# huangjh-pub/di-fusion

Measured on AMD Instinct MI355X. Metric: frames/s integrate+decode+mesh, 640x480 synthetic stream, higher is better.
Workload: dtype f32

## Files before the change

### di_fusion_amd/csrc/kernels_extract.hip.h

```cpp
#pragma once

__device__ __forceinline__ void mark_confident_nbhd(const Geo& g, int lin, float ignore_th, const int64_t* __restrict__ indexer,
                                                    const float* __restrict__ obs, const GridMarks& marks) {
    const uint32_t* bits = marks.bits;
    int ix, iy, iz;
    unlinearize(g, lin, ix, iy, iz);
    int cand[7];
    cand[0] = lin;
    cand[1] = linearize(g, clampi(ix - 1, 0, g.nx - 1), iy, iz);
    cand[2] = linearize(g, clampi(ix + 1, 0, g.nx - 1), iy, iz);
    cand[3] = linearize(g, ix, clampi(iy - 1, 0, g.ny - 1), iz);
    cand[4] = linearize(g, ix, clampi(iy + 1, 0, g.ny - 1), iz);
    cand[5] = linearize(g, ix, iy, clampi(iz - 1, 0, g.nz - 1));
    cand[6] = linearize(g, ix, iy, clampi(iz + 1, 0, g.nz - 1));
    int64_t slot[7];
#pragma unroll
    for (int c = 0; c < 7; ++c) slot[c] = indexer[cand[c]];
    float w[7];
#pragma unroll
    for (int c = 0; c < 7; ++c) w[c] = slot[c] >= 0 ? obs[slot[c]] : ignore_th;
    uint32_t word[7];
#pragma unroll
    for (int c = 0; c < 7; ++c) word[c] = (w[c] > ignore_th) ? bits[cand[c] >> 5] : 0xFFFFFFFFu;
    uint32_t prev[7];
// ... 248 lines not shown
            float xn, yn, zn; int ix, iy, iz;
            bool ok = voxel_of(A.geo, pose_row(A.pose, 0, x, y, z), pose_row(A.pose, 1, x, y, z), pose_row(A.pose, 2, x, y, z), xn, yn, zn, ix, iy, iz);
            int64_t slot = -1;
            if (ok) {
                slot = A.indexer[linearize(A.geo, ix, iy, iz)];
                ok = slot >= 0 && A.obs[slot] > A.ignore_th;
            }
            R.live = ok;
            R.out_idx = row;
            if (ok) {
                R.px = (xn - (float)ix) - 0.5f; R.py = (yn - (float)iy) - 0.5f; R.pz = (zn - (float)iz) - 0.5f;
                lat_row = A.latent + slot * L;
            } else if (half == 1) A.out_std[row] = 0.0f;
        }
    } else {
        const int64_t row = tile * 32 + col;
        R.live = row < n_rows;
        if (R.live) {
            const int64_t p = A.list[row];
            float xn, yn, zn; int ix, iy, iz;
            voxel_of(A.geo, A.xyz[p * 3 + 0], A.xyz[p * 3 + 1], A.xyz[p * 3 + 2], xn, yn, zn, ix, iy, iz);
            R.px = (xn - (float)ix) - 0.5f; R.py = (yn - (float)iy) - 0.5f; R.pz = (zn - (float)iz) - 0.5f;
            lat_row = A.latent + A.indexer[linearize(A.geo, ix, iy, iz)] * L;
            R.out_idx = row;
        }
    }
#pragma unroll
    for (int t = 0; t < 16; ++t) {
        const int k = 2 * t + half;
        float v = 0.0f;
        if (R.live) {
            if (row32) v = row32[k];
            else if (k < L) v = lat_row[k];
            else v = (k == L) ? R.px : ((k == L + 1) ? R.py : R.pz);
        }
        xin[t] = v;
    }
    if constexpr (!DENSE) {
        if (A.mode == 2) {
            unsigned nf = 0;
#pragma unroll
            for (int t = 0; t < 16; ++t) nf |= ((__float_as_uint(xin[t]) & 0x7f800000u) == 0x7f800000u) ? 1u : 0u;
            nf |= (unsigned)__shfl_xor((int)nf, 32);
            R.bad = nf != 0;
        }
    }
    return R;
}

template <bool GRAD, bool DENSE = false>
__global__ void __launch_bounds__(GRAD ? 256 : 512, GRAD ? 1 : 2) k_decode(DecodeArgs A, const float* __restrict__ wblob) {
    extern __shared__ __attribute__((aligned(16))) float lds[];
    if (DENSE && A.zero_word && blockIdx.x == 0 && threadIdx.x == 0) *A.zero_word = 0;
    stage_weights(lds, wblob, DEC_LDS_FLOATS);
    const __amdgpu_buffer_rsrc_t wfwd = make_rsrc(wblob, DEC_FLOATS);
    const __amdgpu_buffer_rsrc_t wbwd = make_rsrc(GRAD ? A.wbwd : wblob, GRAD ? DECB_FLOATS : DEC_FLOATS);
    const int lane = lane_id(), half = lane >> 5, col = lane & 31;
    const int wave = (int)((threadIdx.x >> 6) * gridDim.x + blockIdx.x);
    const int nwaves = (int)(gridDim.x * (blockDim.x >> 6));
    const int res3 = A.lat.res * A.lat.res * A.lat.res;
    const int tiles_per_voxel = (res3 + 31) / 32;
    int64_t n_rows, n_tiles;
    if (A.mode == 0) {
        n_rows = (int64_t)(*A.n_ptr) * res3;
        n_tiles = (int64_t)(*A.n_ptr) * tiles_per_voxel;
    } else {
        n_rows = A.n_ptr ? (int64_t)(*A.n_ptr) : A.n_static;
        n_tiles = (n_rows + 31) / 32;
    }
    for (int64_t tile = wave; tile < n_tiles; tile += nwaves) {
        f16v xin;
        const DecodeRow R = decode_row_input<DENSE>(A, tile, col, half, res3, tiles_per_voxel, n_rows, xin);
        const bool live = R.live;
        const int64_t out_idx = R.out_idx;
        const float px = R.px, py = R.py, pz = R.pz;
        float sdf, sd;
        if (!GRAD && A.mode == 1 && A.fold_table) {
            const int b = live ? A.list[tile * 32 + col] / res3 : 0;
            decoder_tile_folded(lds, wfwd, FoldInitGlobal{A.fold_table + (int64_t)b * 256}, px, py, pz, lane, sdf, sd);
        } else if (GRAD) {
            float gx, gy, gz;
            decoder_tile_grad(lds, wfwd, wbwd, xin, lane, sdf, sd, gx, gy, gz);
            if (live && half == 1) {
                const float gs = R.bad ? __builtin_nanf("") : A.grad_scale;
                A.out_grad[out_idx * 3 + 0] = gx * gs;
                A.out_grad[out_idx * 3 + 1] = gy * gs;
                A.out_grad[out_idx * 3 + 2] = gz * gs;
            }
        } else {
            decoder_tile(lds, wfwd, xin, lane, sdf, sd);
        }
        if (live) {
            if (half == 0) A.out_sdf[out_idx] = R.bad ? __builtin_nanf("") : A.sign * sdf;
            else A.out_std[out_idx] = R.bad ? __builtin_nanf("") : sd;
        }
    }
}

template <bool DENSE = false>
__global__ void __launch_bounds__(512, 1) k_decode_x6(DecodeArgs A, const float* __restrict__ wblob, const float* __restrict__ wu) {
    extern __shared__ __attribute__((aligned(16))) float lds[];
    if (DENSE && A.zero_word && blockIdx.x == 0 && threadIdx.x == 0) *A.zero_word = 0;
    stage_weights(lds, wblob, X6_LDS_BYTES / 4);
    const __amdgpu_buffer_rsrc_t wfwd = make_rsrc(wblob, X6_BYTES / 4);
    const __amdgpu_buffer_rsrc_t wun = make_rsrc(wu, X6U_BYTES / 4);
    const int lane = lane_id(), half = lane >> 5, col = lane & 31;
    const int wave = (int)((threadIdx.x >> 6) * gridDim.x + blockIdx.x);
    const int nwaves = (int)(gridDim.x * (blockDim.x >> 6));
    const int res3 = A.lat.res * A.lat.res * A.lat.res;
    const int tiles_per_voxel = (res3 + 31) / 32;
    int64_t n_rows, n_tiles;
    if (A.mode == 0) {
        n_rows = (int64_t)(*A.n_ptr) * res3;
        n_tiles = (int64_t)(*A.n_ptr) * tiles_per_voxel;
    } else {
        n_rows = A.n_ptr ? (int64_t)(*A.n_ptr) : A.n_static;
        n_tiles = (n_rows + 31) / 32;
    }
    for (int64_t tile = wave; tile < n_tiles; tile += nwaves) {
        f16v xin;
        const DecodeRow R = decode_row_input<DENSE>(A, tile, col, half, res3, tiles_per_voxel, n_rows, xin);
        const bool live = R.live;
        const int64_t out_idx = R.out_idx;
        float sdf, sd;
        decoder_tile_x6(lds, wfwd, wun, xin, lane, sdf, sd);
        if (live) {
            if (half == 0) A.out_sdf[out_idx] = R.bad ? __builtin_nanf("") : A.sign * sdf;
            else A.out_std[out_idx] = R.bad ? __builtin_nanf("") : sd;
        }
    }
}

#ifndef GRAD_X6_THREADS
#define GRAD_X6_THREADS 256
#endif
template <int PF, bool DENSE = false>
__global__ void __launch_bounds__(GRAD_X6_THREADS, 1) k_decode_grad_x6(DecodeArgs A, const float* __restrict__ wblob, const float* __restrict__ wu,
                                                          const float* __restrict__ wb) {
    extern __shared__ __attribute__((aligned(16))) float lds[];
    if (DENSE && A.zero_word && blockIdx.x == 0 && threadIdx.x == 0) *A.zero_word = 0;
    stage_weights(lds, wblob, X6_LDS_BYTES / 4);
    const __amdgpu_buffer_rsrc_t wfwd = make_rsrc(wblob, X6_BYTES / 4);
    const __amdgpu_buffer_rsrc_t wun = make_rsrc(wu, X6U_BYTES / 4);
    const __amdgpu_buffer_rsrc_t wbw = make_rsrc(wb, X6B_BYTES / 4);
    const int lane = lane_id(), half = lane >> 5, col = lane & 31;
    const int wave = (int)((threadIdx.x >> 6) * gridDim.x + blockIdx.x);
    const int nwaves = (int)(gridDim.x * (blockDim.x >> 6));
    const int res3 = A.lat.res * A.lat.res * A.lat.res;
    const int64_t n_rows = A.n_ptr ? (int64_t)(*A.n_ptr) : A.n_static;
    const int64_t n_tiles = (n_rows + 31) / 32;
    for (int64_t tile = wave; tile < n_tiles; tile += nwaves) {
        f16v xin;
        const DecodeRow R = decode_row_input<DENSE>(A, tile, col, half, res3, 1, n_rows, xin);
        float sdf, sd, gx, gy, gz;
        decoder_tile_grad_x6<PF>(lds, wfwd, wun, wbw, xin, lane, sdf, sd, gx, gy, gz);
        if (R.live) {
            if (half == 0) A.out_sdf[R.out_idx] = R.bad ? __builtin_nanf("") : A.sign * sdf;
            else {
                const float gs = R.bad ? __builtin_nanf("") : A.grad_scale;
                A.out_std[R.out_idx] = R.bad ? __builtin_nanf("") : sd;
                A.out_grad[R.out_idx * 3 + 0] = gx * gs;
                A.out_grad[R.out_idx * 3 + 1] = gy * gs;
                A.out_grad[R.out_idx * 3 + 2] = gz * gs;
            }
        }
    }
}

template <int NS>
__device__ __forceinline__ void decode_refine_x6_body(const BatchN<DecodeArgs, NS>& B, int S, const float* __restrict__ wblob) {
    extern __shared__ __attribute__((aligned(16))) float lds[];
    const int lane = lane_id(), half = lane >> 5, col = lane & 31;
    const int wave = __builtin_amdgcn_readfirstlane((int)((threadIdx.x >> 6) * gridDim.x + blockIdx.x));
    const int nwaves = (int)(gridDim.x * (blockDim.x >> 6));
    const Lattice lat = B.s[0].lat;
    const float sign = B.s[0].sign;
    const int res3 = lat.res * lat.res * lat.res, r = lat.res;
    Ranges<NS, int64_t> rg;
    rg.pre[0] = 0;
#pragma unroll
    for (int j = 0; j < NS; ++j) {
        rg.cnt[j] = (j < S) ? (B.s[j].n_ptr ? (int64_t)(*B.s[j].n_ptr) : B.s[j].n_static) : 0;
        rg.pre[j + 1] = rg.pre[j] + (rg.cnt[j] + 31) / 32;
    }
    const int64_t n_tiles = rg.total();
    int sm_n; int64_t lt_n, rows_n;
    rg.locate(wave, sm_n, lt_n, rows_n);
    int e_next = (wave < n_tiles && lt_n * 32 + col < rows_n) ? B.s[sm_n].list[lt_n * 32 + col] : 0;
    __builtin_amdgcn_sched_barrier(0);
    stage_weights(lds, wblob, X6_LDS_BYTES / 4);
    const __amdgpu_buffer_rsrc_t wfwd = make_rsrc(wblob, X6_BYTES / 4);
    for (int64_t T = wave; T < n_tiles; T += nwaves) {
        const int sm = sm_n;
        const int64_t tile = lt_n, n_rows = rows_n;
        const DecodeArgs& A = B.s[sm];
        const int64_t row = tile * 32 + col;
        const bool live = row < n_rows;
        const int e = e_next;
        rg.locate(T + nwaves, sm_n, lt_n, rows_n);
        e_next = (T + nwaves < n_tiles && lt_n * 32 + col < rows_n) ? B.s[sm_n].list[lt_n * 32 + col] : 0;
        const int b = e / res3, sb = e - b * res3;
        const float px = lat.coord(sb / (r * r)), py = lat.coord((sb / r) % r), pz = lat.coord(sb % r);
        float sdf, sd;
// ... 64 lines not shown
                cube_sdf[e0 + jz] = -sv;
                cube_std[e0 + jz] = dv;
                if (fabsf(sv) < 0.05f) sel |= 1u << jz;
            }
        }
        int total;
        int ex = block_excl_scan(__popc(sel), smem, total);
        if (total > 0) {
            if (threadIdx.x == 0) s_base = atomicAdd(counters + DIF_C_VH, total);
            __syncthreads();
            int o = s_base + ex;
            while (sel) {
                int jz = __ffs((int)sel) - 1;
                sel &= sel - 1;
                refine_list[o++] = (int32_t)(e0 + jz);
            }
        }
        __syncthreads();
    }
}

struct VoxelDecodeArgs {
    const int32_t* occ_slot;
    const float* latent;
    Lattice low;
    int R;
    float* cube_sdf;
    float* cube_std;
    int32_t* refine_list;
    int* counters;
    const float* fold_w;
    float* fold_table;
};

#define VD_MAX_L3 64
#define VD_MAX_R2 64
#define VD_WAVE_LDS_FLOATS (2 * VD_MAX_L3 + 2 * 256)

#ifdef DIF_TRACE
__device__ unsigned long long g_vd_trace[2048 * 8];
#define VD_STAMP(slot) do { if (lane_id() == 0) g_vd_trace[((threadIdx.x >> 6) * gridDim.x + blockIdx.x) * 8 + (slot)] = wall_clock64(); } while (0)
#else
#define VD_STAMP(slot) do { } while (0)
#endif

template <bool X6, int NS>
__device__ __forceinline__ void decode_voxels_body(const BatchN<VoxelDecodeArgs, NS>& AB, int S, const float* __restrict__ wblob) {
    extern __shared__ __attribute__((aligned(16))) float lds[];
    VD_STAMP(0);
    constexpr int LDS_W = X6 ? X6_LDS_BYTES / 4 : ((DEC_LDS_FLOATS + 3) & ~3);
#if defined(DIF_VD_CUT) && DIF_VD_CUT == 0
    return;
#endif
    stage_weights(lds, wblob, X6 ? X6_LDS_BYTES / 4 : DEC_LDS_FLOATS);
    VD_STAMP(1);
#if defined(DIF_VD_CUT) && DIF_VD_CUT == 1
    return;
#endif
    const __amdgpu_buffer_rsrc_t wfwd = make_rsrc(wblob, X6 ? X6_BYTES / 4 : DEC_FLOATS);
    const int lane = lane_id(), half = lane >> 5, col = lane & 31, wid = threadIdx.x >> 6;
    const int pair = wid >> 1, tsel = wid & 1;
    float* w_low_sdf = lds + LDS_W + pair * VD_WAVE_LDS_FLOATS;
    float* w_low_std = w_low_sdf + VD_MAX_L3;
    float* w_fold = w_low_std + VD_MAX_L3 + tsel * 256;
    const Lattice low = AB.s[0].low;
    const float* const fold_w = AB.s[0].fold_w;
    const int l = low.res, R = AB.s[0].R, l3 = l * l * l, R2 = R * R, R3 = R2 * R;
    const float scale = (float)(l - 1) / (float)(R - 1);
    int pre[NS + 1];
    pre[0] = 0;
#pragma unroll
    for (int j = 0; j < NS; ++j) pre[j + 1] = pre[j] + ((j < S) ? AB.s[j].counters[DIF_C_B] : 0);
    const int B = pre[NS];
    const int pairs_per_block = (int)(blockDim.x >> 7), n_pairs = (int)gridDim.x * pairs_per_block;
    const int first = __builtin_amdgcn_readfirstlane(pair * (int)gridDim.x + (int)blockIdx.x);
    __shared__ int s_tot[8], s_map[8], s_base[NS];
    const int rounds = (B + n_pairs - 1) / n_pairs;
    for (int round = 0; round < rounds; ++round) {
        const int bg = first + round * n_pairs;
        int sm = 0, b = bg;
#pragma unroll
        for (int j = 1; j < NS; ++j)
            if (bg >= pre[j]) { sm = j; b = bg - pre[j]; }
        const VoxelDecodeArgs& A = AB.s[sm];
        unsigned sel = 0;
        const int jz0 = tsel * (R >> 1), jz1 = jz0 + (R >> 1);
        const int64_t e0 = (int64_t)b * R3 + (int64_t)lane * R;
        if (bg < B && tsel * 32 < l3) {
            const float* lat_row = A.latent + (int64_t)A.occ_slot[b] * L;
            const int s = tsel * 32 + col;
            const float px = low.coord(s / (l * l)), py = low.coord((s / l) % l), pz = low.coord(s % l);
            float sdf = 0.0f, sd = 0.0f;
            if (X6 || fold_w) {
                if constexpr (X6) decoder_fold_consts_x6(lds, fold_w, lat_row, w_fold, lane);
                else decoder_fold_consts(lds, fold_w, lat_row, w_fold, lane);
                __builtin_amdgcn_wave_barrier();
                __builtin_amdgcn_s_waitcnt(0xc07f);
                if (tsel == 0) {
                    float* rec = A.fold_table + (int64_t)b * 256;
                    for (int p = lane; p < 256; p += 64) rec[p] = w_fold[p];
                }
                VD_STAMP(6);
#if defined(DIF_VD_CUT) && DIF_VD_CUT == 2
                sdf = w_fold[lane]; sd = w_fold[lane + 64];
#else
                if constexpr (X6) decoder_tile_folded_x6(lds, wfwd, FoldInitLds{w_fold}, px, py, pz, lane, sdf, sd);
                else decoder_tile_folded(lds, wfwd, FoldInitLds{w_fold}, px, py, pz, lane, sdf, sd);
#endif
            } else if constexpr (!X6) {
                f16v xin;
#pragma unroll
                for (int t = 0; t < 16; ++t) {
                    const int k = 2 * t + half;
                    xin[t] = (k < L) ? lat_row[k] : 0.0f;
                }
                if (half) { xin[14] = px; xin[15] = pz; } else { xin[15] = py; }
                decoder_tile(lds, wfwd, xin, lane, sdf, sd);
            }
            if (s < l3) {
                if (half == 0) w_low_sdf[s] = sdf;
                else w_low_std[s] = sd;
            }
        }
        __syncthreads();
        VD_STAMP(2);
        if (bg < B && lane < R2) {
            const int jx = lane / R, jy = lane % R;
            int x0, x1, y0, y1; float wx0, wx1, wy0, wy1;
            tri_axis(jx, l, scale, x0, x1, wx0, wx1);
            tri_axis(jy, l, scale, y0, y1, wy0, wy1);
            float* const cube_sdf = A.cube_sdf;
            float* const cube_std = A.cube_std;
            for (int jz = jz0; jz < jz1; ++jz) {
                int z0, z1; float wz0, wz1;
                tri_axis(jz, l, scale, z0, z1, wz0, wz1);
                float sv = tri_sample(w_low_sdf, l, x0, x1, y0, y1, z0, z1, wx0, wx1, wy0, wy1, wz0, wz1);
                float dv = tri_sample(w_low_std, l, x0, x1, y0, y1, z0, z1, wx0, wx1, wy0, wy1, wz0, wz1);
                cube_sdf[e0 + jz] = -sv;
                cube_std[e0 + jz] = dv;
                if (fabsf(sv) < 0.05f) sel |= 1u << jz;
            }
        }
        VD_STAMP(3);
        const int c = __popc(sel);
        const int incl = wave_incl_scan(c);
        const int total = __shfl(incl, 63);
        if (lane == 0) { s_tot[wid] = total; if (NS > 1) s_map[wid] = sm; }
        __syncthreads();
        if (NS == 1) {
            if (threadIdx.x == 0) {
                int sum = 0;
                for (int w = 0; w < (int)(blockDim.x >> 6); ++w) sum += s_tot[w];
                s_base[0] = sum ? atomicAdd(A.counters + DIF_C_VH, sum) : 0;
            }
        } else if ((int)threadIdx.x < S) {
            const int j = (int)threadIdx.x;
            int sum = 0;
            for (int w = 0; w < (int)(blockDim.x >> 6); ++w) sum += (s_map[w] == j) ? s_tot[w] : 0;
            s_base[j] = sum ? atomicAdd(AB.s[j].counters + DIF_C_VH, sum) : 0;
        }
        __syncthreads();
        if (total > 0) {
// ... 25 lines not shown
```

### di_fusion_amd/csrc/kernels_optimize.hip.h

```cpp
#pragma once

struct OptimSet {
    const float* obs; const uint8_t* optimized; const int64_t* pos; float enc_th;
    __device__ __forceinline__ bool has(int64_t slot) const { return slot >= 0 && obs[slot] >= enc_th && !optimized[slot] && pos[slot] > 0; }
};

__global__ void __launch_bounds__(DIF_BLOCK) k_optim_focus(Geo g, OptimSet S, const float* __restrict__ xyz, const uint8_t* __restrict__ unq_mask, int64_t N,
                                                         const int64_t* __restrict__ indexer, uint8_t* __restrict__ focus, int* __restrict__ counters) {
    const int64_t i = (int64_t)blockIdx.x * blockDim.x + threadIdx.x;
    if (i == 0) { counters[DIF_C_OPT_ROWS] = 0; counters[DIF_C_OPT_VOXELS] = 0; }
    if (i >= N) return;
    float xn, yn, zn; int ix, iy, iz;
    bool f = false;
    if (unq_mask[i] && voxel_of(g, xyz[i * 3 + 0], xyz[i * 3 + 1], xyz[i * 3 + 2], xn, yn, zn, ix, iy, iz)) {
        const int lin = linearize(g, ix, iy, iz), plane = g.ny * g.nz;
        const int nl[7] = {lin, lin - plane, lin + plane, lin - g.nz, lin + g.nz, lin - 1, lin + 1};
        const bool in_grid[7] = {true, ix > 0, ix < g.nx - 1, iy > 0, iy < g.ny - 1, iz > 0, iz < g.nz - 1};
#pragma unroll
        for (int q = 0; q < 7; ++q) f |= in_grid[q] && S.has(indexer[nl[q]]);
    }
    focus[i] = f ? 1 : 0;
}

struct OptimGatherFunctor {
// ... 6 lines not shown
        i = j - (int64_t)o * N;
        if (!focus[i]) return -1;
        float xn, yn, zn; int ix, iy, iz;
        voxel_of(g, xyz[i * 3 + 0], xyz[i * 3 + 1], xyz[i * 3 + 2], xn, yn, zn, ix, iy, iz);
        const float ox = (o & 4) ? 0.5f : -0.5f, oy = (o & 2) ? 0.5f : -0.5f, oz = (o & 1) ? 0.5f : -0.5f;
        const float gx = fminf(fmaxf(ceilf(xn + ox) - 1.0f, 0.0f), (float)(g.nx - 1));
        const float gy = fminf(fmaxf(ceilf(yn + oy) - 1.0f, 0.0f), (float)(g.ny - 1));
        const float gz = fminf(fmaxf(ceilf(zn + oz) - 1.0f, 0.0f), (float)(g.nz - 1));
        rx = (xn - gx) - 0.5f; ry = (yn - gy) - 0.5f; rz = (zn - gz) - 0.5f;
        const int64_t slot = indexer[linearize(g, (int)gx, (int)gy, (int)gz)];
        return S.has(slot) ? slot : -1;
    }
    __device__ int count(int j) const { float a, b, c; int64_t i; return neighbour(j, a, b, c, i) >= 0 ? 1 : 0; }
    __device__ void emit(int j, int k) const {
        float rx, ry, rz; int64_t i;
        const int64_t slot = neighbour(j, rx, ry, rz, i);
        const float sdf = noise[k] * 0.05f;
        row_slot[k] = (int)slot;
        row_xyz[(int64_t)k * 3 + 0] = rx + sdf * normal[i * 3 + 0];
        row_xyz[(int64_t)k * 3 + 1] = ry + sdf * normal[i * 3 + 1];
        row_xyz[(int64_t)k * 3 + 2] = rz + sdf * normal[i * 3 + 2];
        row_sdf[k] = sdf;
        slot_flag[slot] = 1;
    }
    __device__ void finish(int total) const { counters[DIF_C_OPT_ROWS] = total; }
};

struct OptimUniqueFunctor {
    const int* slot_flag; int* slot_u; int* uniq_slot; int* counters;
    __device__ int count(int s) const { return slot_flag[s] ? 1 : 0; }
    __device__ void emit(int s, int u) const { uniq_slot[u] = s; slot_u[s] = u; }
    __device__ void finish(int total) const { counters[DIF_C_OPT_VOXELS] = total; }
};

#define DIF_OPT_FIX_SCALE 1099511627776.0f

__global__ void __launch_bounds__(DIF_BLOCK) k_optim_init(const int* __restrict__ uniq_slot, const float* __restrict__ latent, float* __restrict__ z,
                                                        float* __restrict__ m, float* __restrict__ v, long long* __restrict__ grad,
                                                        const int* __restrict__ counters) {
    const int n = counters[DIF_C_OPT_VOXELS] * 32;
    for (int e = blockIdx.x * blockDim.x + threadIdx.x; e < n; e += gridDim.x * blockDim.x) {
        const int u = e >> 5, f = e & 31;
        z[e] = f < L ? latent[(int64_t)uniq_slot[u] * L + f] : 0.0f;
        m[e] = 0.0f; v[e] = 0.0f; grad[e] = 0;
    }
}

template <bool X6>
__global__ void __launch_bounds__(256, 1) k_optim_grad(const float* __restrict__ wblob, const float* __restrict__ wbwd_blob, const float* __restrict__ wu_blob, const int* __restrict__ row_slot,
                                                     const float* __restrict__ row_xyz, const float* __restrict__ row_sdf, const int* __restrict__ slot_u,
                                                     const float* __restrict__ z, unsigned long long* __restrict__ grad, float* __restrict__ loss_sum,
                                                     const int* __restrict__ counters) {
    extern __shared__ __attribute__((aligned(16))) float lds[];
    stage_weights(lds, wblob, X6 ? X6_LDS_BYTES / 4 : DEC_LDS_FLOATS);
    const __amdgpu_buffer_rsrc_t wfwd = make_rsrc(wblob, X6 ? X6_BYTES / 4 : DEC_FLOATS), wbwd = make_rsrc(wbwd_blob, X6 ? X6B_BYTES / 4 : DECB_FLOATS);
    const __amdgpu_buffer_rsrc_t wun = make_rsrc(X6 ? wu_blob : wblob, X6 ? X6U_BYTES / 4 : 4);
    const int lane = lane_id(), half = lane >> 5, col = lane & 31;
    const int wave = (int)((threadIdx.x >> 6) * gridDim.x + blockIdx.x), nwaves = (int)(gridDim.x * (blockDim.x >> 6));
    const int n_rows = counters[DIF_C_OPT_ROWS];
    const float inv_n = 1.0f / (float)n_rows;
    const int n_tiles = (n_rows + 31) >> 5;
    for (int tile = wave; tile < n_tiles; tile += nwaves) {
        const int row = tile * 32 + col;
        const bool live = row < n_rows;
        const int u = live ? slot_u[row_slot[row]] : -1;
        const float* zr = z + (int64_t)(live ? u : 0) * 32;
        f16v xin;
#pragma unroll
        for (int t = 0; t < 16; ++t) {
            const int k = 2 * t + half;
            float val = 0.0f;
            if (live) val = k < L ? zr[k] : row_xyz[(int64_t)row * 3 + (k - L)];
            xin[t] = val;
        }
        float sdf, sd, loss;
        f16v gx;
        if constexpr (X6) decoder_tile_nll_grad_x6<GRAD_X6_PF>(lds, wfwd, wun, wbwd, xin, lane, live ? row_sdf[row] : 0.0f, inv_n, sdf, sd, loss, gx);
        else decoder_tile_nll_grad(lds, wfwd, wbwd, xin, lane, live ? row_sdf[row] : 0.0f, inv_n, sdf, sd, loss, gx);
        const int u_prev = __shfl_up(u, 1), u_next = __shfl_down(u, 1);
        const bool run_head = (col == 0) || (u_prev != u), run_tail = (col == 31) || (u_next != u);
        const uint32_t heads32 = (uint32_t)(__ballot(run_head) >> (half * 32));
        const int my_head = 31 - __clz((int)(heads32 & ((2u << col) - 1u)));
#pragma unroll
        for (int r = 0; r < 16; ++r) {
            long long q = live ? __float2ll_rn(gx[r] * DIF_OPT_FIX_SCALE) : 0ll;
            q = seg_incl_scan32(q, col, my_head);
            const int f = (r & 3) + 8 * (r >> 2) + 4 * half;
            if (live && run_tail && f < L) (void)__hip_atomic_fetch_add(grad + (int64_t)u * 32 + f, (unsigned long long)q, __ATOMIC_RELAXED, __HIP_MEMORY_SCOPE_AGENT);
        }
        if (loss_sum) {
            float ls = (live && half == 0) ? loss : 0.0f;
#pragma unroll
            for (int d = 32; d >= 1; d >>= 1) ls += __shfl_xor(ls, d);
            if (lane == 0) atomicAdd(loss_sum, ls);
        }
    }
}

__global__ void __launch_bounds__(DIF_BLOCK) k_optim_adam(float* __restrict__ z, float* __restrict__ m, float* __restrict__ v, long long* __restrict__ grad,
                                                        const int* __restrict__ counters, int iter, float lr, float reg_lambda) {
    const int n_vox = counters[DIF_C_OPT_VOXELS];
    const float inv_n = 1.0f / (float)counters[DIF_C_OPT_ROWS];
    const int grp = (int)((blockIdx.x * blockDim.x + threadIdx.x) >> 5), ngrp = (int)((gridDim.x * blockDim.x) >> 5), f = threadIdx.x & 31;
    const float b1 = 0.9f, b2 = 0.999f, eps = 1e-8f;
    const float step = lr / (1.0f - powf(b1, (float)iter)), bc2 = sqrtf(1.0f - powf(b2, (float)iter));
    for (int u = grp; u < n_vox; u += ngrp) {
        const int e = u * 32 + f;
        const float zf = z[e];
        float g = (float)grad[e] * (1.0f / DIF_OPT_FIX_SCALE);
        grad[e] = 0;
        if (reg_lambda > 0.0f) {
            float nn = f < L ? zf * zf : 0.0f;
// ... 24 lines not shown
```

### di_fusion_amd/csrc/mlp.hip.h

```cpp
#pragma once
#include "common.hip.h"

namespace dif {

typedef float f16v __attribute__((ext_vector_type(16)));
typedef float f4v __attribute__((ext_vector_type(4)));

__device__ __forceinline__ f16v mfma32(float a, float b, f16v c) { return __builtin_amdgcn_mfma_f32_32x32x2f32(a, b, c, 0, 0, 0); }

__device__ __forceinline__ f16v load_bias16(const float* b, int half) {
    const f4v* p = reinterpret_cast<const f4v*>(b + half * 16);
    f4v b0 = p[0], b1 = p[1], b2 = p[2], b3 = p[3];
    f16v r;
    r[0] = b0.x; r[1] = b0.y; r[2] = b0.z; r[3] = b0.w;
    r[4] = b1.x; r[5] = b1.y; r[6] = b1.z; r[7] = b1.w;
    r[8] = b2.x; r[9] = b2.y; r[10] = b2.z; r[11] = b2.w;
    r[12] = b3.x; r[13] = b3.y; r[14] = b3.z; r[15] = b3.w;
    return r;
}

__device__ __forceinline__ float relu1(float x) { return __int_as_float(max(__float_as_int(x), 0)); }
__device__ __forceinline__ f16v relu16(f16v v) {
#pragma unroll
    for (int i = 0; i < 16; ++i) v[i] = relu1(v[i]);
// ... 130 lines not shown
                                             const f16v& xin, int lane, float& sdf, float& stdv) {
    const int half = lane >> 5;
    f16v hx[1];
    hx[0] = xin;
    f16v h0[4];
#pragma unroll
    for (int mb = 0; mb < 4; ++mb) {
        f16v acc = load_bias16(W + DEC_B0 + mb * 32, half);
        acc = block_mm<1>(reinterpret_cast<const f4v*>(W + DEC_A0) + (mb * 4) * 64, hx, acc, lane);
        h0[mb] = relu16(acc);
    }
    f16v h1[4];
#pragma unroll
    for (int mb = 0; mb < 4; ++mb) {
        f16v acc = load_bias16(W + DEC_B1 + mb * 32, half);
        acc = block_mm<4>(reinterpret_cast<const f4v*>(W + DEC_A1) + (mb * 16) * 64, h0, acc, lane);
        h1[mb] = relu16(acc);
    }
    f16v h2x[4];
#pragma unroll
    for (int mb = 0; mb < 3; ++mb) {
        f16v acc = load_bias16(W + DEC_B2 + mb * 32, half);
        acc = block_mm<4>(reinterpret_cast<const f4v*>(W + DEC_A2) + (mb * 16) * 64, h1, acc, lane);
        h2x[mb] = relu16(acc);
    }
    h2x[3] = xin;
    int off3 = DEC_A3 * 4;
    asm volatile("" : "+s"(off3) : : "memory");
    float ps = 0.0f, pu = 0.0f;
#pragma unroll
    for (int mb = 0; mb < 4; ++mb) {
        f16v acc = load_bias16(W + DEC_B3 + mb * 32, half);
        acc = block_mm_src<4>(BufA{Wg, off3 + mb * 16 * 1024}, h2x, acc, lane);
        acc = relu16(acc);
        f16v ws = load_bias16(W + DEC_HW + mb * 32, half);
        f16v wu = load_bias16(W + DEC_HU + mb * 32, half);
#pragma unroll
        for (int r = 0; r < 16; ++r) {
            ps = fmaf(acc[r], ws[r], ps);
            pu = fmaf(acc[r], wu[r], pu);
        }
    }
    ps += __shfl_xor(ps, 32);
    pu += __shfl_xor(pu, 32);
    ps += W[DEC_HB + 0];
    pu += W[DEC_HB + 1];
    sdf = tanhf(ps);
    float sp = (pu > 20.0f) ? pu : log1pf(expf(pu));
    stdv = 0.05f + 0.5f * sp;
}

#define DECF_FLOATS (2 * 29 * 128)

template <int B0, int B3, int UNROLL>
__device__ __forceinline__ void decoder_fold_consts_at(const float* __restrict__ W , const float* __restrict__ fold ,
                                                       const float* __restrict__ lat_row, float* __restrict__ c, int lane) {
    float a0 = W[B0 + lane], a1 = W[B0 + lane + 64], a2 = W[B3 + lane], a3 = W[B3 + lane + 64];
    const f4v* wk = reinterpret_cast<const f4v*>(fold) + lane;
#pragma unroll UNROLL
    for (int k = 0; k < 29; ++k) {
        const float zk = lat_row[k];
        const f4v wv = wk[k * 64];
        a0 = fmaf(wv.x, zk, a0);
        a1 = fmaf(wv.y, zk, a1);
        a2 = fmaf(wv.z, zk, a2);
        a3 = fmaf(wv.w, zk, a3);
    }
    c[lane] = a0;
    c[lane + 64] = a1;
    c[128 + lane] = a2;
    c[128 + lane + 64] = a3;
}
__device__ __forceinline__ void decoder_fold_consts(const float* __restrict__ W, const float* __restrict__ fold, const float* __restrict__ lat_row,
                                                    float* __restrict__ c, int lane) {
    decoder_fold_consts_at<DEC_B0, DEC_B3, 8>(W, fold, lat_row, c, lane);
}

struct FoldInitLds {
    const float* c;
    __device__ __forceinline__ f16v load(int layer, int mb, int half) const { return load_bias16(c + layer * 128 + mb * 32, half); }
};
struct FoldInitGlobal {
    const float* rec;
    __device__ __forceinline__ f16v load(int layer, int mb, int half) const { return load_bias16(rec + layer * 128 + mb * 32, half); }
};

template <class INIT>
__device__ __forceinline__ void decoder_tile_folded(const float* __restrict__ W , __amdgpu_buffer_rsrc_t Wg , const INIT& init,
                                                    float px, float py, float pz, int lane, float& sdf, float& stdv) {
    const int half = lane >> 5;
    const float b14 = half ? px : 0.0f;
    const float b15 = half ? pz : py;
    f16v h0[4];
#pragma unroll
    for (int mb = 0; mb < 4; ++mb) {
        f16v acc = init.load(0, mb, half);
        const f4v a = reinterpret_cast<const f4v*>(W + DEC_A0)[(mb * 4 + 3) * 64 + lane];
        acc = mfma32(a.z, b14, acc);
        acc = mfma32(a.w, b15, acc);
        h0[mb] = relu16(acc);
        __builtin_amdgcn_sched_barrier(0);
    }
    f16v h1[4];
#pragma unroll
    for (int mb = 0; mb < 4; ++mb) {
        f16v acc = load_bias16(W + DEC_B1 + mb * 32, half);
        acc = block_mm<4>(reinterpret_cast<const f4v*>(W + DEC_A1) + (mb * 16) * 64, h0, acc, lane);
        h1[mb] = relu16(acc);
    }
    f16v h2[3];
#pragma unroll
    for (int mb = 0; mb < 3; ++mb) {
        f16v acc = load_bias16(W + DEC_B2 + mb * 32, half);
        acc = block_mm<4>(reinterpret_cast<const f4v*>(W + DEC_A2) + (mb * 16) * 64, h1, acc, lane);
        h2[mb] = relu16(acc);
    }
    int off3 = DEC_A3 * 4;
    asm volatile("" : "+s"(off3) : : "memory");
    float ps = 0.0f, pu = 0.0f;
#pragma unroll
    for (int mb = 0; mb < 4; ++mb) {
        f16v acc = init.load(1, mb, half);
        const BufA src{Wg, off3 + mb * 16 * 1024};
        const f4v ax = src.load(15, lane);
        acc = block_mm_src<3>(src, h2, acc, lane);
        acc = mfma32(ax.z, b14, acc);
        acc = mfma32(ax.w, b15, acc);
        __builtin_amdgcn_sched_barrier(0);
// ... 67 lines not shown
__device__ __forceinline__ void layer_x6(const SRC& A, const f16v* hin, f16v* acc, int lane) {
    constexpr int NS = (KB1 - KB0) * 2 * NMO;
    Tri ring[PF];
#pragma unroll
    for (int i = 0; i < PF; ++i)
        if (i < NS) ring[i] = A.load(i, lane);
    Tri x[2], xn[2];
#pragma unroll
    for (int i = 0; i < 8; ++i) split_pair_into(hin[KB0], i >> 2, i & 3, x[i >> 2]);
#pragma unroll
    for (int kb = KB0; kb < KB1; ++kb) {
#pragma unroll
        for (int s = 0; s < 2; ++s) {
#pragma unroll
            for (int mo = 0; mo < NMO; ++mo) {
                const int u = s * NMO + mo;
                const int t = (kb - KB0) * 2 * NMO + u;
                const Tri a = ring[t % PF];
                if (t + PF < NS) ring[t % PF] = A.load(t + PF, lane);
                if (kb + 1 < KB1) {
                    constexpr int per = (8 + 2 * NMO - 1) / (2 * NMO);
#pragma unroll
                    for (int i = u * per; i < (u + 1) * per && i < 8; ++i) split_pair_into(hin[kb + 1], i >> 2, i & 3, xn[i >> 2]);
                }
                acc[mo] = step_x6(a, x[s], acc[mo]);
                __builtin_amdgcn_sched_barrier(0);
            }
        }
        if (kb + 1 < KB1) { x[0] = xn[0]; x[1] = xn[1]; }
    }
}

#ifndef X6_PF_LDS
#define X6_PF_LDS 2
#endif
#define X6_A0C 0
#define X6_B0 1024
#define X6_B1 1152
#define X6_B2 1280
#define X6_B3 1376
#define X6_HW 1504
#define X6_HU 1632
#define X6_HB 1760
#define X6_A3C 1764
#define X6_AUX_FLOATS 2788
#define X6_L1 (X6_AUX_FLOATS * 4)
#define X6_L2 (X6_L1 + 98304)
#define X6_LDS_BYTES (X6_L2 + 36864)
#define X6_L3 (X6_L2 + 73728)
#define X6_BYTES (X6_L3 + 73728)

__device__ __forceinline__ void decoder_fold_consts_x6(const float* __restrict__ aux , const float* __restrict__ fold ,
                                                       const float* __restrict__ lat_row, float* __restrict__ c, int lane) {
    decoder_fold_consts_at<X6_B0, X6_B3, 15>(aux, fold, lat_row, c, lane);
}

template <class INIT>
__device__ __forceinline__ void decoder_tile_folded_x6(const float* __restrict__ W , __amdgpu_buffer_rsrc_t Wg, const INIT& init,
                                                       float px, float py, float pz, int lane, float& sdf, float& stdv) {
    const int half = lane >> 5;
    const float b14 = half ? px : 0.0f;
    const float b15 = half ? pz : py;
    const char* Wb = reinterpret_cast<const char*>(W);
    f16v h0[4];
#pragma unroll
    for (int mb = 0; mb < 4; ++mb) {
        f16v acc = init.load(0, mb, half);
        const f4v a = reinterpret_cast<const f4v*>(W + X6_A0C)[mb * 64 + lane];
        acc = mfma32(a.z, b14, acc);
        acc = mfma32(a.w, b15, acc);
        h0[mb] = relu16(acc);
    }
    f16v h1[4];
#pragma unroll
    for (int mb = 0; mb < 4; ++mb) h1[mb] = load_bias16(W + X6_B1 + mb * 32, half);
    layer_x6<0, 4, 4, X6_PF_LDS>(LdsX6{reinterpret_cast<const u4v*>(Wb + X6_L1)}, h0, h1, lane);
#pragma unroll
    for (int mb = 0; mb < 4; ++mb) h1[mb] = relu16(h1[mb]);
    f16v h2[3];
#pragma unroll
    for (int mb = 0; mb < 3; ++mb) h2[mb] = load_bias16(W + X6_B2 + mb * 32, half);
    int goff = X6_L2 + 36864;
    asm volatile("" : "+s"(goff) : : "memory");
    layer_x6<0, 2, 3, X6_PF_LDS>(LdsX6{reinterpret_cast<const u4v*>(Wb + X6_L2)}, h1, h2, lane);
    layer_x6<2, 4, 3, 3>(BufX6{Wg, goff}, h1, h2, lane);
#pragma unroll
    for (int mb = 0; mb < 3; ++mb) h2[mb] = relu16(h2[mb]);
    f16v h3[4];
#pragma unroll
    for (int mb = 0; mb < 4; ++mb) h3[mb] = init.load(1, mb, half);
    layer_x6<0, 3, 4, 3>(BufX6{Wg, goff + 36864}, h2, h3, lane);
    float ps = 0.0f, pu = 0.0f;
#pragma unroll
    for (int mb = 0; mb < 4; ++mb) {
        f16v acc = h3[mb];
        const f4v ax = reinterpret_cast<const f4v*>(W + X6_A3C)[mb * 64 + lane];
        acc = mfma32(ax.z, b14, acc);
        acc = mfma32(ax.w, b15, acc);
        acc = relu16(acc);
        f16v ws = load_bias16(W + X6_HW + mb * 32, half);
        f16v wu = load_bias16(W + X6_HU + mb * 32, half);
#pragma unroll
        for (int r = 0; r < 16; ++r) {
            ps = fmaf(acc[r], ws[r], ps);
            pu = fmaf(acc[r], wu[r], pu);
        }
    }
// ... 472 lines not shown
#pragma unroll
    for (int mb = 0; mb < 4; ++mb) {
        f16v acc = load_bias16(W + DEC_B3 + mb * 32, half);
        acc = block_mm_src<4>(BufA{Wg, off3 + mb * 16 * 1024}, h2x, acc, lane);
        acc = relu16_mask(acc, m3[mb]);
        f16v ws = load_bias16(W + DEC_HW + mb * 32, half);
        f16v wu = load_bias16(W + DEC_HU + mb * 32, half);
#pragma unroll
        for (int r = 0; r < 16; ++r) {
            ps = fmaf(acc[r], ws[r], ps);
            pu = fmaf(acc[r], wu[r], pu);
        }
    }
    ps += __shfl_xor(ps, 32);
    pu += __shfl_xor(pu, 32);
    ps += W[DEC_HB + 0];
    pu += W[DEC_HB + 1];
    sdf = tanhf(ps);
    const float sp = (pu > 20.0f) ? pu : log1pf(expf(pu));
    stdv = 0.05f + 0.5f * sp;
    const float g = fminf(fmaxf(gt, -0.2f), 0.2f), mu = fminf(fmaxf(sdf, -0.2f), 0.2f);
    const float diff = g - mu, var = stdv * stdv;
    loss = (logf(stdv) + 0.918938533204672742f + diff * diff / (2.0f * var)) * inv_n;
    const float d_mu = (sdf >= -0.2f && sdf <= 0.2f) ? -diff / var : 0.0f;
    const float d_sigma = 1.0f / stdv - diff * diff / (var * stdv);
    const float a = inv_n * d_mu * (1.0f - sdf * sdf);
    const float b = inv_n * d_sigma * 0.5f * ((pu > 20.0f) ? 1.0f : 1.0f / (1.0f + expf(-pu)));
    f16v g3[4];
#pragma unroll
    for (int mb = 0; mb < 4; ++mb) {
        f16v ws = load_bias16(W + DEC_HW + mb * 32, half);
        f16v wu = load_bias16(W + DEC_HU + mb * 32, half);
        f16v t;
#pragma unroll
        for (int r = 0; r < 16; ++r) t[r] = a * ws[r] + b * wu[r];
        g3[mb] = apply_mask16(t, m3[mb]);
    }
    f16v g2[3];
#pragma unroll
    for (int mb = 0; mb < 3; ++mb)
        g2[mb] = apply_mask16(block_mm_src<4>(BufA{Wb, offb + DECB_T3 * 4 + mb * 16 * 1024}, g3, zero16(), lane), m2[mb]);
    f16v gskip = block_mm_src<4>(BufA{Wb, offb + DECB_T3 * 4 + 3 * 16 * 1024}, g3, zero16(), lane);
    f16v g1[4];
#pragma unroll
    for (int mb = 0; mb < 4; ++mb)
        g1[mb] = apply_mask16(block_mm_src<3>(BufA{Wb, offb + DECB_T2 * 4 + mb * 12 * 1024}, g2, zero16(), lane), m1[mb]);
    f16v g0[4];
#pragma unroll
    for (int mb = 0; mb < 4; ++mb)
        g0[mb] = apply_mask16(block_mm_src<4>(BufA{Wb, offb + DECB_T1 * 4 + mb * 16 * 1024}, g1, zero16(), lane), m0[mb]);
    gx = block_mm_src<4>(BufA{Wb, offb + DECB_T0 * 4}, g0, gskip, lane);
}

__device__ __forceinline__ void stage_weights(float* lds, const float* __restrict__ g, int n_floats) {
    const f4v* __restrict__ src = reinterpret_cast<const f4v*>(g);
    f4v* dst = reinterpret_cast<f4v*>(lds);
    const int n4 = n_floats / 4, step = (int)blockDim.x;
    int i = (int)threadIdx.x;
    for (; i + 7 * step < n4; i += 8 * step) {
        f4v v[8];
#pragma unroll
        for (int k = 0; k < 8; ++k) v[k] = src[i + k * step];
#pragma unroll
        for (int k = 0; k < 8; ++k) dst[i + k * step] = v[k];
    }
    for (; i < n4; i += step) dst[i] = src[i];
    __syncthreads();
}

}
```

Before: 10030.

## Stage decoder weights via async global_load_lds and prefetch latent rows

Weight staging into LDS now uses direct global-to-LDS loads (global_load_lds) instead of round-tripping through registers, split into an issue step and a wait step. The fused decode kernel overlaps this staging with the first latent-row and occupancy-slot fetches, and then software-pipelines the next row's latent fetch across loop iterations. It reads latents via readlane from a per-lane register. Counter reads are hoisted ahead of staging in the other kernels so their latency overlaps too. This adds manual waitcnt and scheduling barriers, which carry correctness risk if the counter encoding is wrong.

```diff
diff --git a/di_fusion_amd/csrc/kernels_extract.hip.h b/di_fusion_amd/csrc/kernels_extract.hip.h
--- a/di_fusion_amd/csrc/kernels_extract.hip.h
+++ b/di_fusion_amd/csrc/kernels_extract.hip.h
@@ -324,12 +324,6 @@
 __global__ void __launch_bounds__(GRAD ? 256 : 512, GRAD ? 1 : 2) k_decode(DecodeArgs A, const float* __restrict__ wblob) {
     extern __shared__ __attribute__((aligned(16))) float lds[];
     if (DENSE && A.zero_word && blockIdx.x == 0 && threadIdx.x == 0) *A.zero_word = 0;
-    stage_weights(lds, wblob, DEC_LDS_FLOATS);
-    const __amdgpu_buffer_rsrc_t wfwd = make_rsrc(wblob, DEC_FLOATS);
-    const __amdgpu_buffer_rsrc_t wbwd = make_rsrc(GRAD ? A.wbwd : wblob, GRAD ? DECB_FLOATS : DEC_FLOATS);
-    const int lane = lane_id(), half = lane >> 5, col = lane & 31;
-    const int wave = (int)((threadIdx.x >> 6) * gridDim.x + blockIdx.x);
-    const int nwaves = (int)(gridDim.x * (blockDim.x >> 6));
     const int res3 = A.lat.res * A.lat.res * A.lat.res;
     const int tiles_per_voxel = (res3 + 31) / 32;
     int64_t n_rows, n_tiles;
@@ -340,6 +334,12 @@
         n_rows = A.n_ptr ? (int64_t)(*A.n_ptr) : A.n_static;
         n_tiles = (n_rows + 31) / 32;
     }
+    stage_weights(lds, wblob, DEC_LDS_FLOATS);
+    const __amdgpu_buffer_rsrc_t wfwd = make_rsrc(wblob, DEC_FLOATS);
+    const __amdgpu_buffer_rsrc_t wbwd = make_rsrc(GRAD ? A.wbwd : wblob, GRAD ? DECB_FLOATS : DEC_FLOATS);
+    const int lane = lane_id(), half = lane >> 5, col = lane & 31;
+    const int wave = (int)((threadIdx.x >> 6) * gridDim.x + blockIdx.x);
+    const int nwaves = (int)(gridDim.x * (blockDim.x >> 6));
     for (int64_t tile = wave; tile < n_tiles; tile += nwaves) {
         f16v xin;
         const DecodeRow R = decode_row_input<DENSE>(A, tile, col, half, res3, tiles_per_voxel, n_rows, xin);
@@ -373,12 +373,6 @@
 __global__ void __launch_bounds__(512, 1) k_decode_x6(DecodeArgs A, const float* __restrict__ wblob, const float* __restrict__ wu) {
     extern __shared__ __attribute__((aligned(16))) float lds[];
     if (DENSE && A.zero_word && blockIdx.x == 0 && threadIdx.x == 0) *A.zero_word = 0;
-    stage_weights(lds, wblob, X6_LDS_BYTES / 4);
-    const __amdgpu_buffer_rsrc_t wfwd = make_rsrc(wblob, X6_BYTES / 4);
-    const __amdgpu_buffer_rsrc_t wun = make_rsrc(wu, X6U_BYTES / 4);
-    const int lane = lane_id(), half = lane >> 5, col = lane & 31;
-    const int wave = (int)((threadIdx.x >> 6) * gridDim.x + blockIdx.x);
-    const int nwaves = (int)(gridDim.x * (blockDim.x >> 6));
     const int res3 = A.lat.res * A.lat.res * A.lat.res;
     const int tiles_per_voxel = (res3 + 31) / 32;
     int64_t n_rows, n_tiles;
@@ -389,6 +383,12 @@
         n_rows = A.n_ptr ? (int64_t)(*A.n_ptr) : A.n_static;
         n_tiles = (n_rows + 31) / 32;
     }
+    stage_weights(lds, wblob, X6_LDS_BYTES / 4);
+    const __amdgpu_buffer_rsrc_t wfwd = make_rsrc(wblob, X6_BYTES / 4);
+    const __amdgpu_buffer_rsrc_t wun = make_rsrc(wu, X6U_BYTES / 4);
+    const int lane = lane_id(), half = lane >> 5, col = lane & 31;
+    const int wave = (int)((threadIdx.x >> 6) * gridDim.x + blockIdx.x);
+    const int nwaves = (int)(gridDim.x * (blockDim.x >> 6));
     for (int64_t tile = wave; tile < n_tiles; tile += nwaves) {
         f16v xin;
         const DecodeRow R = decode_row_input<DENSE>(A, tile, col, half, res3, tiles_per_voxel, n_rows, xin);
@@ -411,6 +411,8 @@
                                                           const float* __restrict__ wb) {
     extern __shared__ __attribute__((aligned(16))) float lds[];
     if (DENSE && A.zero_word && blockIdx.x == 0 && threadIdx.x == 0) *A.zero_word = 0;
+    const int64_t n_rows = A.n_ptr ? (int64_t)(*A.n_ptr) : A.n_static;
+    const int64_t n_tiles = (n_rows + 31) / 32;
     stage_weights(lds, wblob, X6_LDS_BYTES / 4);
     const __amdgpu_buffer_rsrc_t wfwd = make_rsrc(wblob, X6_BYTES / 4);
     const __amdgpu_buffer_rsrc_t wun = make_rsrc(wu, X6U_BYTES / 4);
@@ -419,8 +421,6 @@
     const int wave = (int)((threadIdx.x >> 6) * gridDim.x + blockIdx.x);
     const int nwaves = (int)(gridDim.x * (blockDim.x >> 6));
     const int res3 = A.lat.res * A.lat.res * A.lat.res;
-    const int64_t n_rows = A.n_ptr ? (int64_t)(*A.n_ptr) : A.n_static;
-    const int64_t n_tiles = (n_rows + 31) / 32;
     for (int64_t tile = wave; tile < n_tiles; tile += nwaves) {
         f16v xin;
         const DecodeRow R = decode_row_input<DENSE>(A, tile, col, half, res3, 1, n_rows, xin);
@@ -591,12 +591,6 @@
 #if defined(DIF_VD_CUT) && DIF_VD_CUT == 0
     return;
 #endif
-    stage_weights(lds, wblob, X6 ? X6_LDS_BYTES / 4 : DEC_LDS_FLOATS);
-    VD_STAMP(1);
-#if defined(DIF_VD_CUT) && DIF_VD_CUT == 1
-    return;
-#endif
-    const __amdgpu_buffer_rsrc_t wfwd = make_rsrc(wblob, X6 ? X6_BYTES / 4 : DEC_FLOATS);
     const int lane = lane_id(), half = lane >> 5, col = lane & 31, wid = threadIdx.x >> 6;
     const int pair = wid >> 1, tsel = wid & 1;
     float* w_low_sdf = lds + LDS_W + pair * VD_WAVE_LDS_FLOATS;
@@ -613,6 +607,44 @@
     const int B = pre[NS];
     const int pairs_per_block = (int)(blockDim.x >> 7), n_pairs = (int)gridDim.x * pairs_per_block;
     const int first = __builtin_amdgcn_readfirstlane(pair * (int)gridDim.x + (int)blockIdx.x);
+    const bool has_tile = tsel * 32 < l3;
+    auto locate = [&](int bg, int& sm, int& b) __attribute__((always_inline)) {
+        sm = 0; b = bg;
+#pragma unroll
+        for (int j = 1; j < NS; ++j)
+            if (bg >= pre[j]) { sm = j; b = bg - pre[j]; }
+    };
+    auto request_slot = [&](int bg) __attribute__((always_inline)) {
+        int slot = 0;
+        if (bg < B && has_tile) {
+            int sm, b;
+            locate(bg, sm, b);
+            slot = AB.s[sm].occ_slot[b];
+        }
+        return slot;
+    };
+    auto request_row = [&](int bg, int slot) __attribute__((always_inline)) {
+        float z = 0.0f;
+        if (bg < B && has_tile) {
+            int sm, b;
+            locate(bg, sm, b);
+            const float* row = AB.s[sm].latent + (int64_t)slot * L;
+            if (lane < L) z = row[lane];
+        }
+        return z;
+    };
+    __builtin_amdgcn_sched_barrier(0);
+    const StageTail staged = stage_weights_issue(lds, wblob, X6 ? X6_LDS_BYTES / 4 : DEC_LDS_FLOATS);
+    __builtin_amdgcn_sched_barrier(0);
+    float z_nxt = request_row(first, request_slot(first));
+    int slot_nxt = request_slot(first + n_pairs);
+    __builtin_amdgcn_sched_barrier(0);
+    stage_weights_wait(staged);
+    VD_STAMP(1);
+#if defined(DIF_VD_CUT) && DIF_VD_CUT == 1
+    return;
+#endif
+    const __amdgpu_buffer_rsrc_t wfwd = make_rsrc(wblob, X6 ? X6_BYTES / 4 : DEC_FLOATS);
     __shared__ int s_tot[8], s_map[8], s_base[NS];
     const int rounds = (B + n_pairs - 1) / n_pairs;
     for (int round = 0; round < rounds; ++round) {
@@ -625,14 +657,14 @@
         unsigned sel = 0;
         const int jz0 = tsel * (R >> 1), jz1 = jz0 + (R >> 1);
         const int64_t e0 = (int64_t)b * R3 + (int64_t)lane * R;
-        if (bg < B && tsel * 32 < l3) {
-            const float* lat_row = A.latent + (int64_t)A.occ_slot[b] * L;
+        const LatentLanes z{z_nxt};
+        if (bg < B && has_tile) {
             const int s = tsel * 32 + col;
             const float px = low.coord(s / (l * l)), py = low.coord((s / l) % l), pz = low.coord(s % l);
             float sdf = 0.0f, sd = 0.0f;
             if (X6 || fold_w) {
-                if constexpr (X6) decoder_fold_consts_x6(lds, fold_w, lat_row, w_fold, lane);
-                else decoder_fold_consts(lds, fold_w, lat_row, w_fold, lane);
+                if constexpr (X6) decoder_fold_consts_x6(lds, fold_w, z, w_fold, lane);
+                else decoder_fold_consts(lds, fold_w, z, w_fold, lane);
                 __builtin_amdgcn_wave_barrier();
                 __builtin_amdgcn_s_waitcnt(0xc07f);
                 if (tsel == 0) {
@@ -640,6 +672,9 @@
                     for (int p = lane; p < 256; p += 64) rec[p] = w_fold[p];
                 }
                 VD_STAMP(6);
+                z_nxt = request_row(bg + n_pairs, slot_nxt);
+                slot_nxt = request_slot(bg + 2 * n_pairs);
+                __builtin_amdgcn_sched_barrier(0);
 #if defined(DIF_VD_CUT) && DIF_VD_CUT == 2
                 sdf = w_fold[lane]; sd = w_fold[lane + 64];
 #else
@@ -647,6 +682,7 @@
                 else decoder_tile_folded(lds, wfwd, FoldInitLds{w_fold}, px, py, pz, lane, sdf, sd);
 #endif
             } else if constexpr (!X6) {
+                const float* lat_row = A.latent + (int64_t)A.occ_slot[b] * L;
                 f16v xin;
 #pragma unroll
                 for (int t = 0; t < 16; ++t) {
diff --git a/di_fusion_amd/csrc/kernels_optimize.hip.h b/di_fusion_amd/csrc/kernels_optimize.hip.h
--- a/di_fusion_amd/csrc/kernels_optimize.hip.h
+++ b/di_fusion_amd/csrc/kernels_optimize.hip.h
@@ -82,12 +82,12 @@
                                                      const float* __restrict__ z, unsigned long long* __restrict__ grad, float* __restrict__ loss_sum,
                                                      const int* __restrict__ counters) {
     extern __shared__ __attribute__((aligned(16))) float lds[];
+    const int n_rows = counters[DIF_C_OPT_ROWS];
     stage_weights(lds, wblob, X6 ? X6_LDS_BYTES / 4 : DEC_LDS_FLOATS);
     const __amdgpu_buffer_rsrc_t wfwd = make_rsrc(wblob, X6 ? X6_BYTES / 4 : DEC_FLOATS), wbwd = make_rsrc(wbwd_blob, X6 ? X6B_BYTES / 4 : DECB_FLOATS);
     const __amdgpu_buffer_rsrc_t wun = make_rsrc(X6 ? wu_blob : wblob, X6 ? X6U_BYTES / 4 : 4);
     const int lane = lane_id(), half = lane >> 5, col = lane & 31;
     const int wave = (int)((threadIdx.x >> 6) * gridDim.x + blockIdx.x), nwaves = (int)(gridDim.x * (blockDim.x >> 6));
-    const int n_rows = counters[DIF_C_OPT_ROWS];
     const float inv_n = 1.0f / (float)n_rows;
     const int n_tiles = (n_rows + 31) >> 5;
     for (int tile = wave; tile < n_tiles; tile += nwaves) {
diff --git a/di_fusion_amd/csrc/mlp.hip.h b/di_fusion_amd/csrc/mlp.hip.h
--- a/di_fusion_amd/csrc/mlp.hip.h
+++ b/di_fusion_amd/csrc/mlp.hip.h
@@ -206,19 +206,33 @@
 
 #define DECF_FLOATS (2 * 29 * 128)
 
-template <int B0, int B3, int UNROLL>
+struct LatentRow {
+    const float* row;
+    __device__ __forceinline__ float operator()(int k) const { return row[k]; }
+};
+struct LatentLanes {
+    float v;
+    __device__ __forceinline__ float operator()(int k) const { return __int_as_float(__builtin_amdgcn_readlane(__float_as_int(v), k)); }
+};
+template <int B0, int B3, int UNROLL, class LAT>
 __device__ __forceinline__ void decoder_fold_consts_at(const float* __restrict__ W , const float* __restrict__ fold ,
-                                                       const float* __restrict__ lat_row, float* __restrict__ c, int lane) {
+                                                       const LAT& lat, float* __restrict__ c, int lane) {
     float a0 = W[B0 + lane], a1 = W[B0 + lane + 64], a2 = W[B3 + lane], a3 = W[B3 + lane + 64];
     const f4v* wk = reinterpret_cast<const f4v*>(fold) + lane;
-#pragma unroll UNROLL
-    for (int k = 0; k < 29; ++k) {
-        const float zk = lat_row[k];
-        const f4v wv = wk[k * 64];
-        a0 = fmaf(wv.x, zk, a0);
-        a1 = fmaf(wv.y, zk, a1);
-        a2 = fmaf(wv.z, zk, a2);
-        a3 = fmaf(wv.w, zk, a3);
+#pragma unroll 1
+    for (int k0 = 0; k0 < 29; k0 += UNROLL) {
+#pragma unroll
+        for (int j = 0; j < UNROLL; ++j) {
+            const int k = k0 + j;
+            if (k < 29) {
+                const float zk = lat(k);
+                const f4v wv = wk[k * 64];
+                a0 = fmaf(wv.x, zk, a0);
+                a1 = fmaf(wv.y, zk, a1);
+                a2 = fmaf(wv.z, zk, a2);
+                a3 = fmaf(wv.w, zk, a3);
+            }
+        }
     }
     c[lane] = a0;
     c[lane + 64] = a1;
@@ -227,7 +241,11 @@
 }
 __device__ __forceinline__ void decoder_fold_consts(const float* __restrict__ W, const float* __restrict__ fold, const float* __restrict__ lat_row,
                                                     float* __restrict__ c, int lane) {
-    decoder_fold_consts_at<DEC_B0, DEC_B3, 8>(W, fold, lat_row, c, lane);
+    decoder_fold_consts_at<DEC_B0, DEC_B3, 8>(W, fold, LatentRow{lat_row}, c, lane);
+}
+__device__ __forceinline__ void decoder_fold_consts(const float* __restrict__ W, const float* __restrict__ fold, const LatentLanes& lat,
+                                                    float* __restrict__ c, int lane) {
+    decoder_fold_consts_at<DEC_B0, DEC_B3, 8>(W, fold, lat, c, lane);
 }
 
 struct FoldInitLds {
@@ -401,7 +419,11 @@
 
 __device__ __forceinline__ void decoder_fold_consts_x6(const float* __restrict__ aux , const float* __restrict__ fold ,
                                                        const float* __restrict__ lat_row, float* __restrict__ c, int lane) {
-    decoder_fold_consts_at<X6_B0, X6_B3, 15>(aux, fold, lat_row, c, lane);
+    decoder_fold_consts_at<X6_B0, X6_B3, 15>(aux, fold, LatentRow{lat_row}, c, lane);
+}
+__device__ __forceinline__ void decoder_fold_consts_x6(const float* __restrict__ aux , const float* __restrict__ fold ,
+                                                       const LatentLanes& lat, float* __restrict__ c, int lane) {
+    decoder_fold_consts_at<X6_B0, X6_B3, 15>(aux, fold, lat, c, lane);
 }
 
 template <class INIT>
@@ -980,20 +1002,34 @@
     gx = block_mm_src<4>(BufA{Wb, offb + DECB_T0 * 4}, g0, gskip, lane);
 }
 
-__device__ __forceinline__ void stage_weights(float* lds, const float* __restrict__ g, int n_floats) {
+struct StageTail { f4v v; f4v* dst; };
+__device__ __forceinline__ StageTail stage_weights_issue(float* lds, const float* __restrict__ g, int n_floats) {
     const f4v* __restrict__ src = reinterpret_cast<const f4v*>(g);
     f4v* dst = reinterpret_cast<f4v*>(lds);
-    const int n4 = n_floats / 4, step = (int)blockDim.x;
-    int i = (int)threadIdx.x;
-    for (; i + 7 * step < n4; i += 8 * step) {
-        f4v v[8];
-#pragma unroll
-        for (int k = 0; k < 8; ++k) v[k] = src[i + k * step];
-#pragma unroll
-        for (int k = 0; k < 8; ++k) dst[i + k * step] = v[k];
-    }
-    for (; i < n4; i += step) dst[i] = src[i];
+    const int n4 = n_floats / 4;
+    StageTail T;
+    T.dst = nullptr;
+    T.v = f4v{0.f, 0.f, 0.f, 0.f};
+    const int n_kib = n4 >> 6, tail = n4 & 63;
+    const int nw = (int)(blockDim.x >> 6), wid = __builtin_amdgcn_readfirstlane((int)(threadIdx.x >> 6));
+    const int lane = (int)(threadIdx.x & 63);
+    if ((int)threadIdx.x < tail) {
+        T.v = src[n_kib * 64 + (int)threadIdx.x];
+        T.dst = dst + n_kib * 64 + (int)threadIdx.x;
+    }
+    for (int k = wid; k < n_kib; k += nw)
+        __builtin_amdgcn_global_load_lds((const __attribute__((address_space(1))) void*)(src + k * 64 + lane),
+                                         (__attribute__((address_space(3))) void*)(dst + k * 64), 16, 0, 0);
+    return T;
+}
+__device__ __forceinline__ void stage_weights_wait(const StageTail& T) {
+    if (T.dst) *T.dst = T.v;
+    __builtin_amdgcn_s_waitcnt(0x0f70);
     __syncthreads();
 }
-
-}
+__device__ __forceinline__ void stage_weights(float* lds, const float* __restrict__ g, int n_floats) {
+    const StageTail T = stage_weights_issue(lds, g, n_floats);
+    stage_weights_wait(T);
+}
+
+}
```

Result: no change. 10010 (-0.2%).
